# lrjconan/LanczosNetwork

Hardware: AMD Instinct MI355X
Metric: molecules/sec LanczosNet forward, QM8 batch=1024 (higher is better)
Workload: dtype f32; 1 GPU; QM8 LanczosNet batch=1024/GPU, N<=32 dense L (tile N=26), K=20, fp32, 7x128 layers, 1xMI355X per rank; step = [pack L + batch plan + Lanczos + tridiagonal eigensolver (Ritz pairs)] (one launch) + spectral gains + fused forward; global_batch=1024, parallelism=dp1 (batch shards, async score all-gather per step)

## Files before the change

include/lanczosnet_hip.h:

```cpp
#ifndef LANCZOSNET_HIP_H_
#define LANCZOSNET_HIP_H_

#include <stdint.h>

#ifdef __cplusplus
extern "C" {
#endif

#define LNZ_ABI_VERSION 7
#define LNZ_OK 0
#define LNZ_EINVAL (-1)
#define LNZ_ELAUNCH (-2)
#define LNZ_ENOTSUP (-3)

#define LNZ_TILE 32
#define LNZ_MAX_CHANNELS 32
#define LNZ_STRIP_SUB 6
#define LNZ_STRIP_INTS 80
#define LNZ_STRIP_MAX_B 2048

typedef void* lnz_stream_t;

int lnz_abi_version(void);
const char* lnz_last_error(void);
const char* lnz_last_kernel(void);

int lnz_laplacian_l4(const float* adjs, const int32_t* n_nodes, int B, int N, int E,
                     float* L, lnz_stream_t stream);
int lnz_laplacian(const float* adjs, const int32_t* n_nodes, int B, int N, int E, int kind,
                  double alpha, float* L, lnz_stream_t stream);

int lnz_lanczos_ritz(const float* A, int64_t stride_b, int64_t stride_r, int64_t stride_c,
                     const int32_t* n_nodes, int B, int N, int K, float* D, float* V,
                     int32_t* info, lnz_stream_t stream);
// ... 219 lines not shown
  float* dx0;
  int32_t bwd_din0;
  const float* x0;
  float* msg;
  int32_t msg_layer;
  const uint32_t* ident;
  const int64_t* row_off;
  float* dgains;
  float* dy_compact;
  int64_t dy_compact_rows;
  float* dbias_part;
  int32_t dbias_part_cap;
  const int32_t* strips;
  const int32_t* n_strips;
  int strip_cap;
} lnz_forward_args;
int lnz_lanczosnet_forward(const lnz_forward_args* args, lnz_stream_t stream);
int lnz_lanczosnet_input_grad(const lnz_forward_args* args, lnz_stream_t stream);
int lnz_lanczosnet_gain_grad(const lnz_forward_args* args, lnz_stream_t stream);
int lnz_lanczosnet_messages(const lnz_forward_args* args, lnz_stream_t stream);
int lnz_plan_wg_cap(int B, int n_cu);
int lnz_plan_tiles(const uint8_t* mask, int B, int N, int n_cu, int allow_pairs, int32_t* plan,
                   int32_t* n_wg, lnz_stream_t stream);
int lnz_plan_batch(const uint8_t* mask, int B, int N, int n_cu, int allow_pairs, int32_t* plan,
                   int32_t* n_wg, int K, int32_t* gain_rows, int32_t* n_gain_rows,
                   int32_t* strips, int32_t* n_strips, lnz_stream_t stream);
int lnz_strip_cap(int B);
int lnz_plan_strips(const uint8_t* mask, int B, int N, int n_cu, int32_t* strips,
                    int32_t* n_strips, lnz_stream_t stream);
int64_t lnz_head_backward_workspace_floats(int P, int n_wg);
// ... 120 lines not shown
```

lanczosnet_amd/_lib.py:

```python
import ctypes as C
import os

_HERE = os.path.dirname(os.path.abspath(__file__))
LIB_PATH = os.environ.get('LANCZOSNET_HIP_LIB') or os.path.join(_HERE, 'csrc', 'liblanczosnet_hip.so')

LNZ_OK, LNZ_EINVAL, LNZ_ELAUNCH, LNZ_ENOTSUP = 0, -1, -2, -3
ABI_VERSION = 7


class LnzError(RuntimeError):
  def __init__(self, code, msg):
    super().__init__('lanczosnet_hip error %d: %s' % (code, msg))
    self.code = code


class NotSupported(LnzError, NotImplementedError):
  pass


class ForwardArgs(C.Structure):
  _fields_ = [
      ('B', C.c_int32), ('N', C.c_int32), ('K', C.c_int32),
      ('num_layer', C.c_int32),
      ('din0', C.c_int32), ('dhid', C.c_int32), ('dout', C.c_int32),
      ('n_short', C.c_int32), ('n_long', C.c_int32), ('n_edge', C.c_int32),
      ('short_dist', C.c_int32 * 8),
      ('node_feat', C.c_void_p), ('node_feat_f', C.c_void_p), ('embedding', C.c_void_p),
      ('num_atom', C.c_int32), ('filter_kind', C.c_int32),
      ('mask', C.c_void_p), ('Lp', C.c_void_p), ('V', C.c_void_p), ('G', C.c_void_p),
      ('Wp', C.c_void_p), ('bias', C.c_void_p),
      ('w_off', C.c_int64 * 16), ('b_off', C.c_int64 * 16),
      ('Wp_head', C.c_void_p), ('bias_head', C.c_void_p),
      ('score', C.c_void_p), ('state_out', C.c_void_p),
      ('gemm_mode', C.c_int32), ('plan', C.c_void_p), ('n_wg', C.c_void_p), ('plan_wg_cap', C.c_int),
      ('act_out', C.c_void_p), ('act', C.c_void_p), ('dy', C.c_void_p), ('dx0', C.c_void_p),
      ('bwd_din0', C.c_int32), ('x0', C.c_void_p), ('msg', C.c_void_p), ('msg_layer', C.c_int32), ('ident', C.c_void_p), ('row_off', C.c_void_p), ('dgains', C.c_void_p),
      ('dy_compact', C.c_void_p), ('dy_compact_rows', C.c_int64), ('dbias_part', C.c_void_p),
      ('dbias_part_cap', C.c_int32),
      ('strips', C.c_void_p), ('n_strips', C.c_void_p), ('strip_cap', C.c_int),
  ]


_P, _I, _L = C.c_void_p, C.c_int, C.c_int64
SIGNATURES = {
    'lnz_abi_version': (C.c_int, []),
    'lnz_last_error': (C.c_char_p, []),
    'lnz_last_kernel': (C.c_char_p, []),
    'lnz_laplacian_l4': (C.c_int, [_P, _P, _I, _I, _I, _P, _P]),
    'lnz_laplacian': (C.c_int, [_P, _P, _I, _I, _I, _I, C.c_double, _P, _P]),
    'lnz_lanczos_ritz': (C.c_int, [_P, _L, _L, _L, _P, _I, _I, _I, _P, _P, _P, _P]),
    'lnz_lanczos_ritz_workspace_bytes': (C.c_int64, [_I, _I]),
    'lnz_lanczos_ritz_ws': (C.c_int, [_P, _L, _L, _L, _P, _I, _I, _I, _P, _P, _P, _P, _L, _I, _P]),
    'lnz_tridiag_eigh': (C.c_int, [_P, _P, _I, _I, _P, _P, _P]),
    'lnz_lanczos_ritz_large_workspace_bytes': (C.c_int64, [_I, _I]),
# ... 152 lines not shown
```

lanczosnet_amd/csrc/conv_strip.hip:

```cpp
#include "common.hpp"
#include "conv_tiles.hpp"
#include "wave.hpp"
#include <type_traits>

namespace {

constexpr int P = 136;
constexpr int VBP = 20;
constexpr int HP = 33;
constexpr int MAXMOL = 24;
typedef const __attribute__((address_space(3))) float* lds_cptr;
typedef const __attribute__((address_space(3))) f32x4* lds_c4ptr;

__device__ __forceinline__ f32x4 lds4(lds_cptr p) { return *(lds_c4ptr)p; }
__device__ __forceinline__ f32x4 mfma16(float a, float b, f32x4 c) {
  return __builtin_amdgcn_mfma_f32_16x16x4f32(a, b, c, 0, 0, 0);
}
__device__ __forceinline__ f32x4 splat4(float v) { return f32x4{v, v, v, v}; }

typedef _Float16 f16x8 __attribute__((ext_vector_type(8)));
typedef _Float16 f16x4 __attribute__((ext_vector_type(4)));
__device__ __forceinline__ f32x4 mfma32h(f32x4 a, f32x4 b, f32x4 c) {
  return __builtin_amdgcn_mfma_f32_16x16x32_f16(__builtin_bit_cast(f16x8, a), __builtin_bit_cast(f16x8, b),
                                                c, 0, 0, 0);
// ... 53 lines not shown
    const _Float16* g = reinterpret_cast<const _Float16*>(rowp) + half_at(4 * c4);
    const f16x4 h = *reinterpret_cast<const f16x4*>(g), l = *reinterpret_cast<const f16x4*>(g + 32);
    return f32x4{(float)h[0] + (float)l[0], (float)h[1] + (float)l[1], (float)h[2] + (float)l[2],
                 (float)h[3] + (float)l[3]};
  } else {
    return *reinterpret_cast<const f32x4*>(rowp + 4 * c4);
  }
}

constexpr int VH = 512;
constexpr int strip_lds_floats(int S, int nl, bool half = false) {
  return 2 * S * 16 * P + S * 3 * (half ? VH : 16 * VBP) + 2 * nl * S * 16 + 3 * S * 16 + 3 * MAXMOL + 8;
}


template <int S, int MODE, int FK, bool SHORT, bool HALF>
__device__ __forceinline__ void strip_forward(KArgs& a, const int32_t* __restrict__ ent, float* lds,
                                              const int tid, const int wave) {
  constexpr int R = 16 * S;
  constexpr bool FWD = MODE == 0;
  constexpr bool DIAG = FK == 0;
  static_assert(!HALF || (FWD && DIAG && !SHORT), "split precision: inference forward, diagonal gains, no short channels");
#ifdef LNZ_STRIP_PHASES
  long long ph[8] = {0, 0, 0, 0, 0, 0, 0, 0}, t_all = clock64(), _t0 = t_all;
#define LNZ_PH(i) { const long long _t1 = clock64(); ph[i] += _t1 - _t0; _t0 = _t1; }
#else
#define LNZ_PH(i)
#endif
  const int lane = tid & 63;
  const int j = lane & 15, kq = lane >> 4;
  const int N = a.N, K = a.K, B = a.B;
  const int ns = SHORT ? a.n_short : 0, nl = a.n_long, ne = a.n_edge;
  const int C = ns + nl + ne;
  float* Xs = lds;
  float* Vb = Xs + 2 * R * P;
  float* Gs = Vb + S * 3 * (HALF ? VH : 16 * VBP);
  int* rowinfo = reinterpret_cast<int*>(Gs + 2 * nl * R);
// ... 18 lines not shown
      const int n = mext[i];
      const int rows = n <= 4 ? 4 : (n + 3) & ~3;
      if (tid >= mstart[i] && tid < mstart[i] + rows) own = i;
    }
    rowinfo[tid] = own;
    int ok = 0;
    if (own >= 0) {
      const int lrow = tid - mstart[own];
      ok = (lrow < N && a.mask[(int64_t)mid[own] * N + lrow] != 0) ? 1 : 0;
      if (FWD && a.ident) atomicAnd(&idI[tid >> 4], (int)a.ident[mid[own]]);
    }
    rowok[tid] = ok;
  }
  __syncthreads();

  {
    const int d4 = a.din0 >> 2, total = R * d4;
    constexpr int UN = 3;
    for (int base = tid; base < total; base += 512 * UN) {
      int row[UN], c4[UN];
      bool in[UN], valid[UN];
      int64_t at[UN];
#pragma unroll
      for (int u = 0; u < UN; ++u) {
        const int idx = base + 512 * u;
        in[u] = idx < total;
        row[u] = in[u] ? idx / d4 : 0;
        c4[u] = in[u] ? idx - row[u] * d4 : 0;
        const int own = rowinfo[row[u]];
        const int mol = own >= 0 ? mid[own] : 0, lrow = own >= 0 ? row[u] - mstart[own] : 0;
// ... 231 lines not shown
          for (int r = 0; r < 4; ++r)
            xs_put<HALF>(&Xs[nxt * R * P + (16 * I + 4 * kq + r) * P], 16 * wave + j, Y[I][r]);
      }
      __syncthreads();
    }

    LNZ_PH(1)
    f32x4 Z[S], acur[S], alow[HALF ? S : 1];
    auto load_first = [&](lds_cptr x0) {
#pragma unroll
      for (int I = 0; I < S; ++I) {
        acur[I] = lds4(x0 + 16 * I * P);
        if constexpr (HALF) alow[I] = lds4(x0 + 16 * I * P + 16);
      }
    };
    auto steps4 = [&](lds_cptr xb, lds_cptr x0, auto wrap) {
#pragma unroll
      for (int u = 0; u < 4; ++u) {
        ring[(u + 3) & 3] = wp[(u + 3) * 128];
        f32x4 anext[S];
        const lds_cptr xn = (decltype(wrap)::value && u == 3) ? x0 : xb + 16 * (u + 1);
#pragma unroll
        for (int I = 0; I < S; ++I) anext[I] = lds4(xn + 16 * I * P);
        const float4 bv = ring[u];
#pragma unroll
        for (int I = 0; I < S; ++I) Z[I] = mfma16(acur[I][0], bv.x, Z[I]);
#pragma unroll
        for (int I = 0; I < S; ++I) Z[I] = mfma16(acur[I][1], bv.y, Z[I]);
#pragma unroll
        for (int I = 0; I < S; ++I) Z[I] = mfma16(acur[I][2], bv.z, Z[I]);
#pragma unroll
        for (int I = 0; I < S; ++I) Z[I] = mfma16(acur[I][3], bv.w, Z[I]);
#pragma unroll
        for (int I = 0; I < S; ++I) acur[I] = anext[I];
#pragma unroll
        for (int g = 0; g < S; ++g) {
          __builtin_amdgcn_sched_group_barrier(0x008, 3, 0);
          __builtin_amdgcn_sched_group_barrier(0x100, 1, 0);
          if (g == S - 1) __builtin_amdgcn_sched_group_barrier(0x020, 1, 0);
          __builtin_amdgcn_sched_group_barrier(0x008, 1, 0);
        }
      }
      wp += 4 * 128;
    };
    auto gemm1 = [&](lds_cptr x0, auto&& before_last) {
      if (((chan_total ^ (wave >> 2)) & 1) != 0) __builtin_amdgcn_s_setprio(1);
      else __builtin_amdgcn_s_setprio(0);
      ++chan_total;
#pragma unroll
      for (int I = 0; I < S; ++I) Z[I] = splat4(0.f);
      if constexpr (HALF) {
        before_last();
#pragma unroll
        for (int b = 0; b < 4; ++b) {
          f32x4 anext[S], lnext[S];
          const lds_cptr xn = b == 3 ? x0 : x0 + 32 * (b + 1);
#pragma unroll
          for (int I = 0; I < S; ++I) {
            anext[I] = lds4(xn + 16 * I * P);
            lnext[I] = lds4(xn + 16 * I * P + 16);
          }
          const f32x4 bh = __builtin_bit_cast(f32x4, ring[2 * b]);
          const f32x4 bl = __builtin_bit_cast(f32x4, ring[2 * b + 1]);
// ... 10 lines not shown
            acur[I] = anext[I];
            alow[I] = lnext[I];
          }
        }
        wp += 8 * 128;
        return;
      }
      lds_cptr xb = x0;
#pragma unroll 1
      for (int q0 = 4; q0 < Q16; q0 += 4) {
        steps4(xb, x0, std::false_type{});
        xb += 64;
      }
      before_last();
      steps4(xb, x0, std::true_type{});
    };

    f32x4 mop[S][3];
    auto fetch = [&](int e, bool use_ident) {
#pragma unroll
      for (int I = 0; I < S; ++I) {
        const unsigned skip = (use_ident && ((idm[I] >> e) & 1)) ? OOB : 0u;
#pragma unroll
        for (int d = 0; d < 3; ++d) {
          if (I + d - 1 < 0 || I + d - 1 >= S) continue;
          mop[I][d] = __builtin_bit_cast(
              f32x4, __builtin_amdgcn_raw_buffer_load_b128(l_rsrc, loff[I][d] | skip, e * 4096, 0));
        }
      }
    };
// ... 76 lines not shown
#pragma unroll
          for (int I = 0; I < S; ++I) Z[I] = Zn[I];
        }
        apply_all(out, Z);
      }
    }

    if (nl > 0 && active) {
      const lds_cptr y0 = xlane + nxt * R * P;
      load_first(y0);
      f32x4 T[S];
#pragma unroll
      for (int I = 0; I < S; ++I) T[I] = splat4(0.f);
      for (int s = 0; s < nl; ++s) {
        if constexpr (DIAG) {
          gemm1(y0, [] {});
#pragma unroll
          for (int I = 0; I < S; ++I) {
            const f32x4 gv = *reinterpret_cast<const f32x4*>(gsl + s * R + 16 * I + 4 * kq);
            T[I] += gv * Z[I];
          }
        } else {
          gemm1(y0, [&] {
#pragma unroll
            for (int I = 0; I < S; ++I)
#pragma unroll
              for (int d = 0; d < 3; ++d) {
                if (I + d - 1 < 0 || I + d - 1 >= S) continue;
                mop[I][d] = __builtin_bit_cast(
                    f32x4, __builtin_amdgcn_raw_buffer_load_b128(
                               g_rsrc, doff[DIAG ? 0 : I][d], (la * B * nl + s) * K * K * 4, 0));
// ... 19 lines not shown
#pragma unroll
          for (int r = 0; r < 4; ++r)
#pragma unroll
            for (int I = 0; I < S; ++I) {
              const int J = I + d - 1;
              if (J < 0 || J >= S) continue;
              out[I] = mfma16(vl[I][d][r], T[J][r], out[I]);
            }
      }
    }

    LNZ_PH(3)
    if (active) {
      const lds_cptr x0 = xlane + cur * R * P;
      load_first(x0);
      for (int e = 0; e < ne; ++e) {
        gemm1(x0, [&] { fetch(e, true); });
        LNZ_PH(4)
        apply_all(out, Z);
#pragma unroll
        for (int I = 0; I < S; ++I)
          if ((idm[I] >> e) & 1) out[I] += Z[I];
        LNZ_PH(5)
      }
    }

    if (DIAG && nl > 0 && more) store_gains(lg);
    if (nl > 0) __syncthreads();
    if (active) {
      const int col = 16 * wave + j;
#pragma unroll
      for (int I = 0; I < S; ++I) {
        const int row0 = 16 * I + 4 * kq;
        int own = rowinfo[row0];
        asm volatile("" : "+v"(own));
        const int mol = own >= 0 ? mid[own] : 0;
        const int lrow0 = own >= 0 ? row0 - mstart[own] : 0;
        const int64_t rowbase = (int64_t)mol * 32 + lrow0;
// ... 648 lines not shown
  const int tid = threadIdx.x;
  const int wave = __builtin_amdgcn_readfirstlane(tid >> 6);
  const int32_t* ent = a.strips + (int64_t)blockIdx.x * LNZ_STRIP_INTS;
  const int sub = __builtin_amdgcn_readfirstlane(ent[1]);
  switch (sub) {
    case 1: strip_forward<1, MODE, FK, SHORT, HALF>(a, ent, lds_strip, tid, wave); break;
    case 2: strip_forward<2, MODE, FK, SHORT, HALF>(a, ent, lds_strip, tid, wave); break;
    case 3: strip_forward<3, MODE, FK, SHORT, HALF>(a, ent, lds_strip, tid, wave); break;
    case 4: strip_forward<4, MODE, FK, SHORT, HALF>(a, ent, lds_strip, tid, wave); break;
    case 5: strip_forward<5, MODE, FK, SHORT, HALF>(a, ent, lds_strip, tid, wave); break;
    case 6: strip_forward<6, MODE, FK, SHORT, HALF>(a, ent, lds_strip, tid, wave); break;
    default: break;
  }
}

}

namespace lnz {

bool strip_forward_eligible(const lnz_forward_args& a, int mode) {
  if (mode != 0 && mode != 1) return false;
  if (!a.strips || !a.n_strips || a.strip_cap <= 0) return false;
  if (a.filter_kind != 0 && a.filter_kind != 1) return false;
  if (a.gemm_mode == 1 ? (mode != 0 || a.act_out || a.filter_kind != 0 || a.din0 != 128 || a.n_short != 0)
                       : a.gemm_mode != 0)
    return false;
  if (a.dhid != 128 || a.din0 % 64 != 0 || a.din0 > 128) return false;
  if (mode == 1 && (a.din0 != 128 || a.bwd_din0 % 16 != 0)) return false;
  if (mode == 1 && a.dbias_part &&
      a.strip_cap > (a.dbias_part_cap > 0 ? a.dbias_part_cap : (a.plan ? 2 * a.plan_wg_cap : 0)))
    return false;
  if (a.n_short + a.n_long + a.n_edge > 32 || a.n_edge < 1 || a.n_long > 12 || a.dout > 31) return false;
  if (a.filter_kind == 1 && a.K % 4 != 0) return false;
// ... 30 lines not shown
  LNZ_DYNAMIC_LDS(fn, 160 * 1024, "conv_strip.hip");
  lnz_forward_args args = a;
  void* params[] = {&args};
  (void)hipLaunchKernel(fn, dim3(a.strip_cap), dim3(512), params, bytes, s);
  return check_launch("lnz_lanczosnet_messages (strips)");
}

int launch_strip_gain_grad(const lnz_forward_args& a, hipStream_t s) {
  const size_t bytes = (size_t)strip_lds_floats(LNZ_STRIP_SUB, a.n_long) * sizeof(float);
  LNZ_DYNAMIC_LDS(lanczosnet_strip_gain_grad_kernel, 160 * 1024, "conv_strip.hip");
  hipLaunchKernelGGL(lanczosnet_strip_gain_grad_kernel, dim3(a.strip_cap), dim3(512), bytes, s, a);
  return check_launch("lnz_lanczosnet_gain_grad (strips)");
}

int launch_strip_forward(const lnz_forward_args& a, int mode, hipStream_t s) {
  const size_t bytes = (size_t)strip_lds_floats(LNZ_STRIP_SUB, a.n_long, a.gemm_mode == 1) * sizeof(float);
  const void* fns[8] = {
      (const void*)lanczosnet_strip_kernel<0, 0, false>, (const void*)lanczosnet_strip_kernel<1, 0, false>,
      (const void*)lanczosnet_strip_kernel<0, 2, false>, (const void*)lanczosnet_strip_kernel<1, 2, false>,
      (const void*)lanczosnet_strip_kernel<0, 0, true>,  (const void*)lanczosnet_strip_kernel<1, 0, true>,
      (const void*)lanczosnet_strip_kernel<0, 2, true>,  (const void*)lanczosnet_strip_kernel<1, 2, true>};
  const int which = (a.n_short > 0 ? 4 : 0) + (a.filter_kind == 0 ? 0 : 2) + mode;
  const void* fn = fns[which];
  if (a.gemm_mode == 1) fn = (const void*)lanczosnet_strip_kernel<0, 0, false, true>;
  note_kernel("lanczosnet_strip_kernel<%d,%d,%s,%s>", mode, a.filter_kind == 0 ? 0 : 2,
              a.n_short > 0 && a.gemm_mode != 1 ? "true" : "false", a.gemm_mode == 1 ? "true" : "false");
  LNZ_DYNAMIC_LDS(fn, 160 * 1024, "conv_strip.hip");
  lnz_forward_args args = a;
  void* params[] = {&args};
  (void)hipLaunchKernel(fn, dim3(a.strip_cap), dim3(512), params, bytes, s);
  return check_launch(mode == 0 ? "lnz_lanczosnet_forward (strips)" : "lnz_lanczosnet_input_grad (strips)");
// ... 4 lines not shown
```

lanczosnet_amd/csrc/torch_ext.cpp:

```cpp
#include <ATen/ATen.h>
#include <ATen/hip/impl/HIPStreamMasqueradingAsCUDA.h>
#include <c10/core/DeviceGuard.h>
#include <torch/library.h>

#include <tuple>
#include <vector>

#include "../../include/lanczosnet_hip.h"

namespace {

using at::Tensor;

void check(int code, const char* what) {
  TORCH_CHECK(code == LNZ_OK, what, ": lanczosnet_hip error ", code, ": ", lnz_last_error());
}

lnz_stream_t cur_stream() {
  return (lnz_stream_t)c10::hip::getCurrentHIPStreamMasqueradingAsCUDA().stream();
}

void need(const Tensor& t, at::ScalarType dt, const char* name, bool contiguous = true) {
  TORCH_CHECK(t.is_cuda(), "lanczosnet: ", name, " must be a HIP (cuda) tensor; there is no CPU path");
  TORCH_CHECK(t.scalar_type() == dt, "lanczosnet: ", name, " must be ", dt, ", got ", t.scalar_type());
// ... 18 lines not shown
}
void* raw_any(const c10::optional<Tensor>& t, const char* name) {
  if (!t.has_value()) return nullptr;
  TORCH_CHECK(t->is_cuda(), "lanczosnet: ", name, " must be a HIP (cuda) tensor; there is no CPU path");
  return t->data_ptr();
}
const Tensor* first_defined(std::initializer_list<const Tensor*> ts) {
  for (const Tensor* t : ts)
    if (t && t->defined()) return t;
  return nullptr;
}

#include "torch_ext_abi.inc"

enum { kNodeFeat, kNodeFeatF, kEmbedding, kMask, kLp, kV, kG, kWp, kBias, kWpHead, kBiasHead,
       kPlan, kNwg, kAct, kX0, kIdent, kRowOff, kStrips, kNStrips, kNumIn };
enum { dB, dN, dK, dNumLayer, dDin0, dDhid, dDout, dNLong, dNEdge, dNumAtom, dFilterKind, dGemmMode,
       dPlanCap, dBwdDin0, dMsgLayer, dDyCompactRows, dStripCap, kNumDim };
void fused_launch(int64_t which, const c10::List<c10::optional<Tensor>>& in, at::IntArrayRef dims,
                  at::IntArrayRef w_off, at::IntArrayRef b_off,
                  at::IntArrayRef short_dist, const c10::optional<Tensor>& score,
                  const c10::optional<Tensor>& state_out, const c10::optional<Tensor>& act_out,
                  const c10::optional<Tensor>& dy, const c10::optional<Tensor>& dx0,
                  const c10::optional<Tensor>& msg, const c10::optional<Tensor>& dgains,
                  const c10::optional<Tensor>& dy_compact, const c10::optional<Tensor>& dbias_part) {
  TORCH_CHECK((int)in.size() == kNumIn && (int)dims.size() == kNumDim && which >= 0 && which <= 3,
              "lanczosnet::fused_launch: ", (int)kNumIn, " operands and ", (int)kNumDim, " dims expected");
  TORCH_CHECK(w_off.size() <= 16 && b_off.size() <= 16 && short_dist.size() <= 8);
  auto opt = [&](int i) -> c10::optional<Tensor> { return in.get(i); };
  const c10::optional<Tensor> v = opt(kV);
  TORCH_CHECK(v.has_value() && v->dim() == 3, "lanczosnet::fused_launch: V [B,N,K] is required");
  lnz_forward_args a = {};
  a.B = dims[dB], a.N = dims[dN], a.K = dims[dK], a.num_layer = dims[dNumLayer];
// ... 15 lines not shown
  a.V = (const float*)raw_ptr(v, at::kFloat, "V");
  a.G = (const float*)raw_ptr(opt(kG), at::kFloat, "G");
  a.Wp = (const float*)raw_ptr(opt(kWp), at::kFloat, "Wp");
  a.bias = (const float*)raw_ptr(opt(kBias), at::kFloat, "bias");
  a.Wp_head = (const float*)raw_ptr(opt(kWpHead), at::kFloat, "Wp_head");
  a.bias_head = (const float*)raw_ptr(opt(kBiasHead), at::kFloat, "bias_head");
  a.plan = (const int32_t*)raw_ptr(opt(kPlan), at::kInt, "plan");
  a.n_wg = (const int32_t*)raw_ptr(opt(kNwg), at::kInt, "n_wg");
  a.act = (const float*)raw_ptr(opt(kAct), at::kFloat, "act");
  a.x0 = (const float*)raw_ptr(opt(kX0), at::kFloat, "x0");
  a.ident = (const uint32_t*)raw_ptr(opt(kIdent), at::kInt, "ident");
  a.row_off = (const int64_t*)raw_ptr(opt(kRowOff), at::kLong, "row_off");
  a.strips = (const int32_t*)raw_ptr(opt(kStrips), at::kInt, "strips");
  a.n_strips = (const int32_t*)raw_ptr(opt(kNStrips), at::kInt, "n_strips");
  a.strip_cap = dims[dStripCap];
  if (a.strips)
    TORCH_CHECK(a.n_strips && a.strip_cap > 0 &&
                    opt(kStrips)->numel() >= (int64_t)a.strip_cap * LNZ_STRIP_INTS,
                "lanczosnet::fused_launch: strips shorter than strip_cap entries, or n_strips missing");
  if (a.mask) TORCH_CHECK(opt(kMask)->numel() == (int64_t)a.B * a.N, "lanczosnet::fused_launch: mask is not [B,N]");
  if (a.node_feat) TORCH_CHECK(opt(kNodeFeat)->numel() == (int64_t)a.B * a.N, "lanczosnet::fused_launch: node_feat is not [B,N]");
  if (a.node_feat_f)
    TORCH_CHECK(opt(kNodeFeatF)->numel() == (int64_t)a.B * a.N * a.din0, "lanczosnet::fused_launch: node_feat is not [B,N,din0]");
  if (a.G)
    TORCH_CHECK(opt(kG)->numel() == (int64_t)a.num_layer * a.B * a.n_long * a.K * (a.filter_kind == 1 ? a.K : 1) ||
                    opt(kG)->numel() == (int64_t)a.num_layer * a.B * a.n_long * a.K,
                "lanczosnet::fused_launch: G does not match (num_layer, B, n_long, K[, K])");
  if (a.plan) TORCH_CHECK(opt(kPlan)->numel() >= 12 * (int64_t)a.plan_wg_cap, "lanczosnet::fused_launch: plan shorter than 12 * cap");
  a.score = (float*)raw_ptr(score, at::kFloat, "score");
  a.state_out = (float*)raw_ptr(state_out, at::kFloat, "state_out");
// ... 330 lines not shown
```

lanczosnet_amd/ops.py:

```python
import torch

import os
import threading

from . import _lib, _torch_ext



def _map_error(e):
  msg = str(e)
  if 'lanczosnet_hip error ' not in msg:
    return e
  tail = msg.split('lanczosnet_hip error ', 1)[1]
  try:
    code = int(tail.split(':', 1)[0])
  except ValueError:
    return e
  text = tail.split(':', 1)[1].strip() if ':' in tail else tail
  text = text.split('\nException raised from', 1)[0].strip()
  if code == _lib.LNZ_ENOTSUP:
    return _lib.NotSupported(code, text)
  return _lib.LnzError(code, text)


# ... 1386 lines not shown
    strips, scap = _strip_buf(B, mask_u8.device)
    buf.strips = strips
    _abi().plan_batch(mask_u8, B, N, n_cu, 1, buf, buf[12 * cap:], 0, None, None, strips,
                      strips[scap * STRIP_INTS:])
    return buf, cap
  _abi().plan_tiles(mask_u8, B, N, n_cu, int(bool(allow_pairs)), buf,
                                buf[12 * cap:])
  return buf, cap


def pairing_supported(plan):
  return True


def lanczosnet_forward(plan, node_feat, Lp, V, G, mask, return_state=False, tiling='auto',
                       act_out=None, use_ident=True):
  _need_cuda(node_feat, Lp, V, G, mask)
  B, N, K = V.shape
  ready = getattr(Lp, 'ready', None)
  if ready is not None:
    torch.cuda.current_stream(Lp.device).wait_event(ready)
  if plan.get('gemm_mode', 0) == 1:
    Lp = split_laplacian_pack(Lp)
  elif Lp.dtype != torch.float32:
    raise RuntimeError('this Laplacian pack is the float16 form of a split-precision plan (gemm_mode 1): '
                       'the exact kernels read the fp32 pack')
  if act_out is None and not return_state:
    return _forward_ext(plan, node_feat, Lp, V, G, mask, tiling, use_ident)
  ops_, dims = _fused_operands(plan, V)
  emb = None
  if node_feat.dtype in (torch.int64,):
    ops_[_IN['node_feat']] = node_feat.contiguous()
    emb = ops_[_IN['embedding']] = plan['embedding']
    dims[_DIM['num_atom']] = emb.shape[0]
  else:
    nf = node_feat.to(torch.float32)
    if nf.shape[-1] != plan['din0']:
      assert nf.shape[-1] == plan['din0_raw']
      nf = torch.nn.functional.pad(nf, (0, plan['din0'] - nf.shape[-1]))
    ops_[_IN['node_feat_f']] = nf.contiguous()
  mask_u8 = mask.to(torch.uint8).contiguous()
  ops_[_IN['mask']] = mask_u8
  ops_[_IN['Lp']] = Lp
  ident = getattr(Lp, 'ident', None)
  if ident is not None and use_ident:
    ops_[_IN['ident']] = ident
  fk = int(plan.get('filter_kind', 0))
  if G is not None:
    want = (plan['num_layer'], B, plan['n_long'], K) + ((K,) if fk == 1 else ())
    assert tuple(G.shape) == want and G.is_contiguous() and G.dtype == torch.float32, \
        (tuple(G.shape), want)
  ops_[_IN['G']] = G
  ops_[_IN['Wp']], ops_[_IN['bias']] = plan['Wp'], plan['bias']
  ops_[_IN['Wp_head']], ops_[_IN['bias_head']] = plan['Wp_head'], plan['bias_head']
  gemm_mode = int(plan.get('gemm_mode', 0))
  dims[_DIM['gemm_mode']] = gemm_mode
  if isinstance(tiling, tuple):
    tiles, cap = tiling
  elif tiling != 'none':
    assert tiling in ('auto', 'single')
    tiles, cap = plan_tiles(mask_u8, allow_pairs=(tiling == 'auto' and pairing_supported(plan)))
  if tiling != 'none':
    _set_plan(ops_, dims, tiles, cap)
  if gemm_mode == 1 and ops_[_IN['strips']] is None:
    strips = plan_strips(mask_u8)
    scap = (strips.numel() - 1) // STRIP_INTS
    ops_[_IN['strips']], ops_[_IN['n_strips']] = strips, strips[scap * STRIP_INTS:]
    dims[_DIM['strip_cap']] = scap
  score = torch.empty((B, plan['dout']), dtype=torch.float32, device=V.device)
  if act_out is not None:
    assert tuple(act_out.shape) == (plan['num_layer'], B, 32, plan['dhid']) and \
        act_out.is_contiguous() and act_out.dtype == torch.float32
  state = None
  if return_state:
    state = torch.zeros((B, 32, plan['dhid']), dtype=torch.float32, device=V.device)
  nl = plan['num_layer']
  _ext().fused_launch(0, ops_, dims, [int(x) for x in plan['w_off'][:nl]],
                      [int(x) for x in plan['b_off'][:nl]], [int(p) for p in plan['short']],
                      score, state, act_out, None, None, None, None, None, None)
  return (score, state) if return_state else score


_IN = {k: i for i, k in enumerate(
    ['node_feat', 'node_feat_f', 'embedding', 'mask', 'Lp', 'V', 'G', 'Wp', 'bias', 'Wp_head',
     'bias_head', 'plan', 'n_wg', 'act', 'x0', 'ident', 'row_off',
     'strips', 'n_strips'])}
_DIM = {k: i for i, k in enumerate(
    ['B', 'N', 'K', 'num_layer', 'din0', 'dhid', 'dout', 'n_long', 'n_edge', 'num_atom', 'filter_kind',
     'gemm_mode', 'plan_cap', 'bwd_din0', 'msg_layer', 'dy_compact_rows', 'strip_cap'])}


def _fused_operands(plan, V):
  B, N, K = V.shape
  ops_ = [None] * len(_IN)
  ops_[_IN['V']] = _f32c(V)
  dims = [0] * len(_DIM)
  for k, v in (('B', B), ('N', N), ('K', K), ('num_layer', plan['num_layer']), ('din0', plan['din0']),
               ('dhid', plan['dhid']), ('dout', plan['dout']), ('n_long', plan['n_long']),
               ('n_edge', plan['n_edge']), ('filter_kind', int(plan.get('filter_kind', 0)))):
    dims[_DIM[k]] = int(v)
  return ops_, dims


def _set_plan(ops_, dims, tiles, cap):
  ops_[_IN['plan']] = tiles
  ops_[_IN['n_wg']] = tiles[12 * cap:]
  dims[_DIM['plan_cap']] = int(cap)
  strips = getattr(tiles, 'strips', None)
  if strips is not None:
    scap = (strips.numel() - 1) // STRIP_INTS
    ops_[_IN['strips']], ops_[_IN['n_strips']] = strips, strips[scap * STRIP_INTS:]
    dims[_DIM['strip_cap']] = scap


STRIP_INTS = 80


def strip_plan_wanted(B, N):
  return N <= 32


def _strip_buf(B, device):
  scap = _abi().strip_cap(B)
  return torch.empty((scap * STRIP_INTS + 1,), dtype=torch.int32, device=device), scap


def plan_strips(mask_u8, n_cu=None):
  B, N = mask_u8.shape
  n_cu = n_cu or _n_cu(mask_u8.device)
  buf, scap = _strip_buf(B, mask_u8.device)
# ... 477 lines not shown
```

lanczosnet_amd/utils/flop_model.py:

```python
import numpy as np

FLOP_PER_MFMA = 2 * 32 * 32 * 2
FLOP_PER_MFMA16 = 2 * 16 * 16 * 4
FLOP_PER_MOPS_COUNT = 512


def _row_groups(n_a, n_b, split):
  ga = (n_a + 7) >> 3
  gb = ((n_b + 7) >> 3) if n_b > 0 else 0
  return ga + gb if split < 32 else ga


def _subtiles16(n_a, n_b, split):
  mask = (1 << ((n_a + 7) >> 3)) - 1
  if split < 32 and n_b > 0:
    mask |= ((1 << ((n_b + 7) >> 3)) - 1) << (split >> 3)
  return (1 if mask & 3 else 0) + (1 if mask & 12 else 0)


def forward16_selected(cfg):
  hid = cfg['hidden_dim']
  return (len(cfg['short_diffusion_dist']) == 0 and all(h == 128 for h in hid) and
          cfg['input_dim'] % 64 == 0 and cfg['input_dim'] <= 128 and
          len(cfg['long_diffusion_dist']) <= 12)
# ... 148 lines not shown
      useful += (din0 // 16) * 4 * touched
    issued += S * 64
    useful += S * 64
    full = issued
    rows_real += t['rows_real']
    rows_tile += 16 * S
  return dict(tiles=len(strips), mfma_issued=int(issued), mfma_unskipped=int(full),
              flops_issued=int(issued) * FLOP_PER_MFMA16, flops_unskipped=int(full) * FLOP_PER_MFMA16,
              mops_counts=int(issued) * (FLOP_PER_MFMA16 // FLOP_PER_MOPS_COUNT),
              useful_row_frac=rows_real / float(max(1, rows_tile)),
              mfma_in_touched_blocks=int(useful),
              subtiles=int(sum(t['sub'] for t in strips)),
              max_subtiles_per_strip=int(max(t['sub'] for t in strips)))


FLOP_PER_MFMA16X32_F16 = 2 * 16 * 16 * 32


def strip_split_mfma_issued(strips, cfg):
  n_long = len(cfg['long_diffusion_dist'])
  n_edge = cfg['num_bond_type'] + 1
  C = n_long + n_edge
  nl = cfg['num_layer']

  def pairs(S):
    n = 0
    for I in range(S):
      p0 = max(I - 1, 0) >> 1
      n += 1
      if 2 * (p0 + 1) < S and 2 * (p0 + 1) <= I + 1:
# ... 15 lines not shown
```

Measured before the change: 1.342 million molecules/s.

## Fold sparse rare edge channels into one shared GEMM plus low-rank corrections

Adds a strip kernel variant that, per strip, scans the rare edge-type Laplacian channels (channels 2 and up) to find rows that differ from identity. When few rows are touched, it sums the weights of those channels and runs one folded GEMM against X, then adds sparse corrections for the touched rows as 'virtual subtiles' built in LDS. The goal is to skip the full per-channel GEMM and block products for nearly empty bond-type channels. The cost is a per-strip scan of the Laplacian tiles, extra LDS, and a different kernel instantiation; S=6 strips fall back to the old path.

```diff
diff --git a/include/lanczosnet_hip.h b/include/lanczosnet_hip.h
--- a/include/lanczosnet_hip.h
+++ b/include/lanczosnet_hip.h
@@ -18,6 +18,7 @@
 #define LNZ_STRIP_SUB 6
 #define LNZ_STRIP_INTS 80
 #define LNZ_STRIP_MAX_B 2048
+#define LNZ_RARE_DEBUG_INTS 512
 
 typedef void* lnz_stream_t;
 
@@ -267,6 +268,9 @@
   const int32_t* strips;
   const int32_t* n_strips;
   int strip_cap;
+  int32_t* rare_strips;
+  int32_t no_fold;
+  int32_t* rare_debug;
 } lnz_forward_args;
 int lnz_lanczosnet_forward(const lnz_forward_args* args, lnz_stream_t stream);
 int lnz_lanczosnet_input_grad(const lnz_forward_args* args, lnz_stream_t stream);
diff --git a/lanczosnet_amd/_lib.py b/lanczosnet_amd/_lib.py
--- a/lanczosnet_amd/_lib.py
+++ b/lanczosnet_amd/_lib.py
@@ -38,6 +38,7 @@
       ('dy_compact', C.c_void_p), ('dy_compact_rows', C.c_int64), ('dbias_part', C.c_void_p),
       ('dbias_part_cap', C.c_int32),
       ('strips', C.c_void_p), ('n_strips', C.c_void_p), ('strip_cap', C.c_int),
+      ('rare_strips', C.c_void_p), ('no_fold', C.c_int32), ('rare_debug', C.c_void_p),
   ]
 
 
diff --git a/lanczosnet_amd/csrc/conv_strip.hip b/lanczosnet_amd/csrc/conv_strip.hip
--- a/lanczosnet_amd/csrc/conv_strip.hip
+++ b/lanczosnet_amd/csrc/conv_strip.hip
@@ -91,13 +91,19 @@
 }
 
 
-template <int S, int MODE, int FK, bool SHORT, bool HALF>
+constexpr int RARE_MAXV = 8, RARE_MAXF = 5, RARE_MAXS = 5;
+constexpr int rare_lds_floats(int S) {
+  return RARE_MAXV * S * 256 + RARE_MAXV * 16 + 2 * RARE_MAXV + 8 + RARE_MAXF * 16 * S + 8;
+}
+
+template <int S, int MODE, int FK, bool SHORT, bool HALF, bool RARE = false>
 __device__ __forceinline__ void strip_forward(KArgs& a, const int32_t* __restrict__ ent, float* lds,
                                               const int tid, const int wave) {
   constexpr int R = 16 * S;
   constexpr bool FWD = MODE == 0;
   constexpr bool DIAG = FK == 0;
   static_assert(!HALF || (FWD && DIAG && !SHORT), "split precision: inference forward, diagonal gains, no short channels");
+  static_assert(!RARE || (FWD && DIAG && !SHORT && !HALF && S <= RARE_MAXS), "rare form: exact inference forward, S <= 5");
 #ifdef LNZ_STRIP_PHASES
   long long ph[8] = {0, 0, 0, 0, 0, 0, 0, 0}, t_all = clock64(), _t0 = t_all;
 #define LNZ_PH(i) { const long long _t1 = clock64(); ph[i] += _t1 - _t0; _t0 = _t1; }
@@ -146,6 +152,143 @@
   }
   __syncthreads();
 
+  float* rx = lds + strip_lds_floats(S, nl);
+  f32x4* Af = reinterpret_cast<f32x4*>(rx);
+  int* vsrc = reinterpret_cast<int*>(rx + RARE_MAXV * S * 256);
+  int* vchan = vsrc + RARE_MAXV * 16;
+  int* tcnt = vchan + 2 * RARE_MAXV;
+  int* tlist = tcnt + 8;
+  int* rflag = tlist + RARE_MAXF * R;
+  bool rare = false;
+  int nvs = 0;
+  if constexpr (RARE) {
+    const int NF = ne - 2;
+    constexpr int TCAP = RARE_MAXF * MAXMOL;
+    unsigned* tmask = reinterpret_cast<unsigned*>(rx);
+    int* tiles = reinterpret_cast<int*>(tmask + TCAP);
+    int* ntile = tiles + TCAP;
+    if (tid < TCAP) tmask[tid] = 0u;
+    if (tid < 2) ntile[tid] = 0;
+    __syncthreads();
+    if (tid < nm * NF) {
+      const int own = tid / NF, f = tid - own * NF;
+      if (a.ident && ((a.ident[mid[own]] >> (2 + f)) & 1u)) tiles[TCAP - 1 - atomicAdd(ntile + 1, 1)] = own * 8 + f;
+      else tiles[atomicAdd(ntile, 1)] = own * 8 + f;
+    }
+    __syncthreads();
+    {
+      const int whole = ntile[0] * 256, total = whole + ntile[1] * 32;
+      constexpr int UN = 4;
+      for (int base = tid; base < total; base += 512 * UN) {
+        float4 v[UN];
+        int tl[UN], o[UN];
+#pragma unroll
+        for (int u = 0; u < UN; ++u) {
+          const int idx = base + 512 * u;
+          tl[u] = -1, o[u] = 0;
+          if (idx < whole) {
+            tl[u] = tiles[idx >> 8], o[u] = idx & 255;
+          } else if (idx < total) {
+            const int jd = idx - whole, r = jd & 31;
+            tl[u] = tiles[TCAP - 1 - (jd >> 5)], o[u] = (r >> 3) * 64 + ((r >> 2) & 1) * 32 + r;
+          }
+          const int64_t at = tl[u] >= 0 ? ((int64_t)mid[tl[u] >> 3] * ne + 2 + (tl[u] & 7)) * 256 + o[u] : 0;
+          v[u] = reinterpret_cast<const float4*>(a.Lp)[at];
+        }
+#pragma unroll
+        for (int u = 0; u < UN; ++u) {
+          if (tl[u] < 0) continue;
+          const int own = tl[u] >> 3;
+          const int row = o[u] & 31, col0 = 8 * (o[u] >> 6) + 4 * ((o[u] >> 5) & 1);
+          const float x[4] = {v[u].x, v[u].y, v[u].z, v[u].w};
+          const int n = mext[own], rows_own = n <= 4 ? 4 : (n + 3) & ~3;
+          unsigned bits = 0u;
+#pragma unroll
+          for (int c = 0; c < 4; ++c) {
+            if (col0 + c != row) bits |= x[c] != 0.0f ? (1u << row) | (1u << (col0 + c)) : 0u;
+            else if (row < rows_own && x[c] != (rowok[mstart[own] + row] != 0 ? 1.0f : 0.0f)) bits |= 1u << row;
+          }
+          if (bits) atomicOr(&tmask[(tl[u] & 7) * MAXMOL + own], bits);
+        }
+      }
+    }
+    __syncthreads();
+    if (wave < NF) {
+      int base = 0;
+      for (int h = 0; h < 2; ++h) {
+        const int row = lane + 64 * h;
+        bool t = false;
+        if (row < R) {
+          const int own = rowinfo[row];
+          if (own >= 0) t = (tmask[wave * MAXMOL + own] >> (row - mstart[own])) & 1;
+        }
+        const unsigned long long m = __ballot(t);
+        if (t) tlist[wave * R + base + __popcll(m & ((1ull << lane) - 1ull))] = row;
+        base += __popcll(m);
+      }
+      if (lane == 0) tcnt[wave] = base;
+    }
+    __syncthreads();
+    if (tid == 0) {
+      int nv = 0;
+      for (int f = 0; f < NF; ++f)
+        for (int s0 = 0; s0 < tcnt[f]; s0 += 16) {
+          if (nv < RARE_MAXV) vchan[nv] = 2 + f, vchan[RARE_MAXV + nv] = s0;
+          ++nv;
+        }
+      const int folded = 32 * S + nv * (32 + 4 * S), plain = (32 * S + 4 * (3 * S - 2)) * NF;
+      rflag[0] = (nv <= RARE_MAXV && folded < plain) ? 1 : 0;
+      rflag[1] = nv;
+    }
+    __syncthreads();
+    rare = __builtin_amdgcn_readfirstlane(rflag[0]) != 0;
+    nvs = rare ? __builtin_amdgcn_readfirstlane(rflag[1]) : 0;
+    if (a.rare_debug) {
+      int32_t* dbg = a.rare_debug + (int64_t)blockIdx.x * LNZ_RARE_DEBUG_INTS;
+      if (tid == 0) dbg[0] = rflag[0], dbg[1] = rflag[1];
+      if (tid < NF) dbg[2 + tid] = tcnt[tid];
+      if (tid < RARE_MAXV && tid < rflag[1]) dbg[8 + tid] = vchan[tid];
+      for (int idx = tid; idx < NF * R; idx += 512) {
+        const int f = idx / R, i = idx - f * R;
+        if (i < tcnt[f]) dbg[16 + 96 * f + i] = tlist[idx];
+      }
+    }
+    if (rare) {
+      if (tid == 0 && a.rare_strips) atomicAdd(a.rare_strips, 1);
+      if (tid < nvs * 16) {
+        const int v = tid >> 4, f = vchan[v] - 2, s0 = vchan[RARE_MAXV + v], slot = s0 + (tid & 15);
+        vsrc[tid] = tlist[f * R + (slot < tcnt[f] ? slot : s0)];
+      }
+      __syncthreads();
+      for (int idx = tid; idx < nvs * S * 64; idx += 512) {
+        const int v = idx / (S * 64), rem = idx - v * (S * 64);
+        const int I = rem >> 6, jj = rem & 15, kk = (rem >> 4) & 3;
+        const int e = vchan[v], f = e - 2, s0 = vchan[RARE_MAXV + v];
+        const int p = 16 * I + jj, own = rowinfo[p];
+        float val[4];
+        bool ok[4];
+        int q[4];
+#pragma unroll
+        for (int r = 0; r < 4; ++r) {
+          const int slot = 4 * kk + r;
+          q[r] = vsrc[v * 16 + slot];
+          ok[r] = s0 + slot < tcnt[f] && own >= 0 && rowinfo[q[r]] == own;
+          int64_t at = 0;
+          if (ok[r]) {
+            const int st = mstart[own], lp = p - st, lq = q[r] - st;
+            at = ((((int64_t)mid[own] * ne + e) * 256 + (lq >> 3) * 64 + ((lq >> 2) & 1) * 32 + lp) << 2) + (lq & 3);
+          }
+          val[r] = a.Lp[at];
+        }
+        f32x4 d;
+#pragma unroll
+        for (int r = 0; r < 4; ++r)
+          d[r] = ok[r] ? val[r] - ((q[r] == p && rowok[p] != 0) ? 1.0f : 0.0f) : 0.0f;
+        Af[idx] = d;
+      }
+    }
+  }
+
   {
     const int d4 = a.din0 >> 2, total = R * d4;
     constexpr int UN = 3;
@@ -407,10 +550,32 @@
         if constexpr (HALF) alow[I] = lds4(x0 + 16 * I * P + 16);
       }
     };
+    const float4* __restrict__ wnext = wp;
+    const float4* __restrict__ wjump = nullptr;
+    f32x4 wf[8];
+    float4 wft[RARE_MAXF];
+    int gi = 0;
+    auto fold_load = [&](int q) {
+#pragma unroll
+      for (int f = 0; f < RARE_MAXF; ++f) {
+        const int e = 2 + f < ne ? 2 + f : ne - 1;
+        wft[f] = Wl[((int64_t)rt * Gtot + (int64_t)(ns + nl + e) * Q) * 64 + wlane + q * 128];
+      }
+    };
+    auto fold_add = [&](int q) {
+      f32x4 sum = splat4(0.f);
+#pragma unroll
+      for (int f = 0; f < RARE_MAXF; ++f)
+        if (2 + f < ne) sum += f32x4{wft[f].x, wft[f].y, wft[f].z, wft[f].w};
+#pragma unroll
+      for (int qq = 0; qq < 8; ++qq)
+        if (qq == q) wf[qq] = sum;
+    };
     auto steps4 = [&](lds_cptr xb, lds_cptr x0, auto wrap) {
 #pragma unroll
       for (int u = 0; u < 4; ++u) {
-        ring[(u + 3) & 3] = wp[(u + 3) * 128];
+        if (RARE && decltype(wrap)::value && u >= 1) ring[(u + 3) & 3] = wnext[(u - 1) * 128];
+        else ring[(u + 3) & 3] = wp[(u + 3) * 128];
         f32x4 anext[S];
         const lds_cptr xn = (decltype(wrap)::value && u == 3) ? x0 : xb + 16 * (u + 1);
 #pragma unroll
@@ -440,6 +605,10 @@
       if (((chan_total ^ (wave >> 2)) & 1) != 0) __builtin_amdgcn_s_setprio(1);
       else __builtin_amdgcn_s_setprio(0);
       ++chan_total;
+      if constexpr (RARE) {
+        wnext = wjump ? wjump : wp + Q16 * 128;
+        wjump = nullptr;
+      }
 #pragma unroll
       for (int I = 0; I < S; ++I) Z[I] = splat4(0.f);
       if constexpr (HALF) {
@@ -480,6 +649,14 @@
       }
       before_last();
       steps4(xb, x0, std::true_type{});
+      if constexpr (RARE) wp = wnext;
+    };
+    auto gemm1_carry = [&](lds_cptr x0, auto&& before_last) {
+      const bool carry = RARE && rare && gi < Q16;
+      if (carry) fold_load(gi);
+      gemm1(x0, before_last);
+      if (carry) fold_add(gi);
+      ++gi;
     };
 
     f32x4 mop[S][3];
@@ -586,7 +763,8 @@
       for (int I = 0; I < S; ++I) T[I] = splat4(0.f);
       for (int s = 0; s < nl; ++s) {
         if constexpr (DIAG) {
-          gemm1(y0, [] {});
+          if constexpr (RARE) gemm1_carry(y0, [] {});
+          else gemm1(y0, [] {});
 #pragma unroll
           for (int I = 0; I < S; ++I) {
             const f32x4 gv = *reinterpret_cast<const f32x4*>(gsl + s * R + 16 * I + 4 * kq);
@@ -636,14 +814,94 @@
     if (active) {
       const lds_cptr x0 = xlane + cur * R * P;
       load_first(x0);
-      for (int e = 0; e < ne; ++e) {
-        gemm1(x0, [&] { fetch(e, true); });
+      const int ne_plain = (RARE && rare) ? 2 : ne;
+      auto wchan = [&](int v) {
+        const int e = __builtin_amdgcn_readfirstlane(vchan[v]);
+        return Wl + ((int64_t)rt * Gtot + (int64_t)(ns + nl + e) * Q) * 64 + wlane;
+      };
+      for (int e = 0; e < ne_plain; ++e) {
+        if constexpr (RARE) {
+          if (rare && e == 1 && nvs > 0) wjump = wchan(0);
+          gemm1_carry(x0, [&] { fetch(e, true); });
+        } else {
+          gemm1(x0, [&] { fetch(e, true); });
+        }
         LNZ_PH(4)
         apply_all(out, Z);
 #pragma unroll
         for (int I = 0; I < S; ++I)
           if ((idm[I] >> e) & 1) out[I] += Z[I];
         LNZ_PH(5)
+      }
+      if constexpr (RARE) {
+        if (rare) {
+          for (int q = gi; q < Q16; ++q) {
+            fold_load(q);
+            fold_add(q);
+          }
+          if (((chan_total ^ (wave >> 2)) & 1) != 0) __builtin_amdgcn_s_setprio(1);
+          else __builtin_amdgcn_s_setprio(0);
+          ++chan_total;
+#pragma unroll
+          for (int I = 0; I < S; ++I) Z[I] = splat4(0.f);
+#pragma unroll
+          for (int q = 0; q < 8; ++q) {
+            if (q < Q16) {
+              f32x4 av[S];
+#pragma unroll
+              for (int I = 0; I < S; ++I) av[I] = lds4(x0 + 16 * q + 16 * I * P);
+#pragma unroll
+              for (int c = 0; c < 4; ++c)
+#pragma unroll
+                for (int I = 0; I < S; ++I) Z[I] = mfma16(av[I][c], wf[q][c], Z[I]);
+            }
+          }
+#pragma unroll
+          for (int I = 0; I < S; ++I) {
+            const int4 okv = *reinterpret_cast<const int4*>(rowok + 16 * I + 4 * kq);
+            out[I][0] += okv.x ? Z[I][0] : 0.0f;
+            out[I][1] += okv.y ? Z[I][1] : 0.0f;
+            out[I][2] += okv.z ? Z[I][2] : 0.0f;
+            out[I][3] += okv.w ? Z[I][3] : 0.0f;
+          }
+          LNZ_PH(4)
+          for (int v = 0; v < nvs; ++v) {
+            if (((chan_total ^ (wave >> 2)) & 1) != 0) __builtin_amdgcn_s_setprio(1);
+            else __builtin_amdgcn_s_setprio(0);
+            ++chan_total;
+            const float4* __restrict__ wn = v + 1 < nvs ? wchan(v + 1) : wp;
+            const lds_cptr xa = (lds_cptr)(Xs + cur * R * P + vsrc[v * 16 + j] * P + 4 * kq);
+            f32x4 zg[4] = {splat4(0.f), splat4(0.f), splat4(0.f), splat4(0.f)};
+            f32x4 ac = lds4(xa);
+#pragma unroll 1
+            for (int q0 = 0; q0 < Q16; q0 += 4) {
+              const bool last = q0 + 4 >= Q16;
+#pragma unroll
+              for (int u = 0; u < 4; ++u) {
+                const float4* pf = (last && u >= 1) ? wn + (u - 1) * 128 : wp + (u + 3) * 128;
+                ring[(u + 3) & 3] = *pf;
+                const f32x4 an = lds4(xa + 16 * ((q0 + u + 1) & (Q16 - 1)));
+                const float4 bv = ring[u];
+                zg[0] = mfma16(ac[0], bv.x, zg[0]);
+                zg[1] = mfma16(ac[1], bv.y, zg[1]);
+                zg[2] = mfma16(ac[2], bv.z, zg[2]);
+                zg[3] = mfma16(ac[3], bv.w, zg[3]);
+                ac = an;
+              }
+              wp += 4 * 128;
+            }
+            wp = wn;
+            const f32x4 zs = (zg[0] + zg[1]) + (zg[2] + zg[3]);
+            f32x4 fr[S];
+#pragma unroll
+            for (int I = 0; I < S; ++I) fr[I] = Af[(v * S + I) * 64 + lane];
+#pragma unroll
+            for (int r = 0; r < 4; ++r)
+#pragma unroll
+              for (int I = 0; I < S; ++I) out[I] = mfma16(fr[I][r], zs[r], out[I]);
+          }
+          LNZ_PH(5)
+        }
       }
     }
 
@@ -1322,9 +1580,37 @@
   }
 }
 
+template <int MODE, int FK, int RARE, bool SHORT, bool HALF>
+__global__ __launch_bounds__(512) void lanczosnet_strip_kernel(const lnz_forward_args) {
+  static_assert(MODE == 0 && FK == 0 && RARE == 1 && !SHORT && !HALF, "one instantiation");
+  KArgs& a = *(KArgs*)__builtin_amdgcn_kernarg_segment_ptr();
+  extern __shared__ __attribute__((aligned(16))) float lds_strip[];
+  if ((int)blockIdx.x >= *a.n_strips) return;
+  const int tid = threadIdx.x;
+  const int wave = __builtin_amdgcn_readfirstlane(tid >> 6);
+  const int32_t* ent = a.strips + (int64_t)blockIdx.x * LNZ_STRIP_INTS;
+  const int sub = __builtin_amdgcn_readfirstlane(ent[1]);
+  switch (sub) {
+    case 1: strip_forward<1, 0, 0, false, false, true>(a, ent, lds_strip, tid, wave); break;
+    case 2: strip_forward<2, 0, 0, false, false, true>(a, ent, lds_strip, tid, wave); break;
+    case 3: strip_forward<3, 0, 0, false, false, true>(a, ent, lds_strip, tid, wave); break;
+    case 4: strip_forward<4, 0, 0, false, false, true>(a, ent, lds_strip, tid, wave); break;
+    case 5: strip_forward<5, 0, 0, false, false, true>(a, ent, lds_strip, tid, wave); break;
+    case 6: strip_forward<6, 0, 0, false, false>(a, ent, lds_strip, tid, wave); break;
+    default: break;
+  }
+}
+
 }
 
 namespace lnz {
+
+static bool strip_rare_eligible(const lnz_forward_args& a, int mode) {
+  if (mode != 0 || a.act_out || a.no_fold) return false;
+  if (a.gemm_mode != 0 || a.filter_kind != 0 || a.n_short != 0) return false;
+  if (a.n_edge < 3 || a.n_edge - 2 > RARE_MAXF) return false;
+  return (size_t)(strip_lds_floats(RARE_MAXS, a.n_long) + rare_lds_floats(RARE_MAXS)) * sizeof(float) <= 160 * 1024;
+}
 
 bool strip_forward_eligible(const lnz_forward_args& a, int mode) {
   if (mode != 0 && mode != 1) return false;
@@ -1385,7 +1671,19 @@
 }
 
 int launch_strip_forward(const lnz_forward_args& a, int mode, hipStream_t s) {
-  const size_t bytes = (size_t)strip_lds_floats(LNZ_STRIP_SUB, a.n_long, a.gemm_mode == 1) * sizeof(float);
+  size_t bytes = (size_t)strip_lds_floats(LNZ_STRIP_SUB, a.n_long, a.gemm_mode == 1) * sizeof(float);
+  if (strip_rare_eligible(a, mode)) {
+    const size_t rb = (size_t)(strip_lds_floats(RARE_MAXS, a.n_long) + rare_lds_floats(RARE_MAXS)) * sizeof(float);
+    bytes = rb > bytes ? rb : bytes;
+    void (*kfn)(const lnz_forward_args) = lanczosnet_strip_kernel<0, 0, 1, false, false>;
+    const void* fn = (const void*)kfn;
+    note_kernel("lanczosnet_strip_kernel<0,0,1,false,false>");
+    LNZ_DYNAMIC_LDS(fn, 160 * 1024, "conv_strip.hip");
+    lnz_forward_args args = a;
+    void* params[] = {&args};
+    (void)hipLaunchKernel(fn, dim3(a.strip_cap), dim3(512), params, bytes, s);
+    return check_launch("lnz_lanczosnet_forward (strips, folded rare channels)");
+  }
   const void* fns[8] = {
       (const void*)lanczosnet_strip_kernel<0, 0, false>, (const void*)lanczosnet_strip_kernel<1, 0, false>,
       (const void*)lanczosnet_strip_kernel<0, 2, false>, (const void*)lanczosnet_strip_kernel<1, 2, false>,
diff --git a/lanczosnet_amd/csrc/torch_ext.cpp b/lanczosnet_amd/csrc/torch_ext.cpp
--- a/lanczosnet_amd/csrc/torch_ext.cpp
+++ b/lanczosnet_amd/csrc/torch_ext.cpp
@@ -56,9 +56,9 @@
 #include "torch_ext_abi.inc"
 
 enum { kNodeFeat, kNodeFeatF, kEmbedding, kMask, kLp, kV, kG, kWp, kBias, kWpHead, kBiasHead,
-       kPlan, kNwg, kAct, kX0, kIdent, kRowOff, kStrips, kNStrips, kNumIn };
+       kPlan, kNwg, kAct, kX0, kIdent, kRowOff, kStrips, kNStrips, kRareStrips, kRareDebug, kNumIn };
 enum { dB, dN, dK, dNumLayer, dDin0, dDhid, dDout, dNLong, dNEdge, dNumAtom, dFilterKind, dGemmMode,
-       dPlanCap, dBwdDin0, dMsgLayer, dDyCompactRows, dStripCap, kNumDim };
+       dPlanCap, dBwdDin0, dMsgLayer, dDyCompactRows, dStripCap, dNoFold, kNumDim };
 void fused_launch(int64_t which, const c10::List<c10::optional<Tensor>>& in, at::IntArrayRef dims,
                   at::IntArrayRef w_off, at::IntArrayRef b_off,
                   at::IntArrayRef short_dist, const c10::optional<Tensor>& score,
@@ -104,6 +104,12 @@
   a.strips = (const int32_t*)raw_ptr(opt(kStrips), at::kInt, "strips");
   a.n_strips = (const int32_t*)raw_ptr(opt(kNStrips), at::kInt, "n_strips");
   a.strip_cap = dims[dStripCap];
+  a.rare_strips = (int32_t*)raw_ptr(opt(kRareStrips), at::kInt, "rare_strips");
+  a.no_fold = (int32_t)dims[dNoFold];
+  a.rare_debug = (int32_t*)raw_ptr(opt(kRareDebug), at::kInt, "rare_debug");
+  if (a.rare_debug)
+    TORCH_CHECK(opt(kRareDebug)->numel() >= (int64_t)dims[dStripCap] * LNZ_RARE_DEBUG_INTS,
+                "lanczosnet::fused_launch: rare_debug shorter than strip_cap * LNZ_RARE_DEBUG_INTS");
   if (a.strips)
     TORCH_CHECK(a.n_strips && a.strip_cap > 0 &&
                     opt(kStrips)->numel() >= (int64_t)a.strip_cap * LNZ_STRIP_INTS,
diff --git a/lanczosnet_amd/ops.py b/lanczosnet_amd/ops.py
--- a/lanczosnet_amd/ops.py
+++ b/lanczosnet_amd/ops.py
@@ -1424,7 +1424,8 @@
 
 
 def lanczosnet_forward(plan, node_feat, Lp, V, G, mask, return_state=False, tiling='auto',
-                       act_out=None, use_ident=True):
+                       act_out=None, use_ident=True, rare_strips=None, fold=True,
+                       rare_debug=None):
   _need_cuda(node_feat, Lp, V, G, mask)
   B, N, K = V.shape
   ready = getattr(Lp, 'ready', None)
@@ -1435,7 +1436,7 @@
   elif Lp.dtype != torch.float32:
     raise RuntimeError('this Laplacian pack is the float16 form of a split-precision plan (gemm_mode 1): '
                        'the exact kernels read the fp32 pack')
-  if act_out is None and not return_state:
+  if act_out is None and not return_state and rare_strips is None and rare_debug is None and fold:
     return _forward_ext(plan, node_feat, Lp, V, G, mask, tiling, use_ident)
   ops_, dims = _fused_operands(plan, V)
   emb = None
@@ -1455,6 +1456,12 @@
   ident = getattr(Lp, 'ident', None)
   if ident is not None and use_ident:
     ops_[_IN['ident']] = ident
+  if rare_strips is not None:
+    assert rare_strips.dtype == torch.int32 and rare_strips.numel() >= 1
+    ops_[_IN['rare_strips']] = rare_strips
+  if rare_debug is not None:
+    assert rare_debug.dtype == torch.int32 and rare_debug.is_contiguous()
+    ops_[_IN['rare_debug']] = rare_debug
   fk = int(plan.get('filter_kind', 0))
   if G is not None:
     want = (plan['num_layer'], B, plan['n_long'], K) + ((K,) if fk == 1 else ())
@@ -1465,6 +1472,7 @@
   ops_[_IN['Wp_head']], ops_[_IN['bias_head']] = plan['Wp_head'], plan['bias_head']
   gemm_mode = int(plan.get('gemm_mode', 0))
   dims[_DIM['gemm_mode']] = gemm_mode
+  dims[_DIM['no_fold']] = 0 if fold else 1
   if isinstance(tiling, tuple):
     tiles, cap = tiling
   elif tiling != 'none':
@@ -1494,10 +1502,10 @@
 _IN = {k: i for i, k in enumerate(
     ['node_feat', 'node_feat_f', 'embedding', 'mask', 'Lp', 'V', 'G', 'Wp', 'bias', 'Wp_head',
      'bias_head', 'plan', 'n_wg', 'act', 'x0', 'ident', 'row_off',
-     'strips', 'n_strips'])}
+     'strips', 'n_strips', 'rare_strips', 'rare_debug'])}
 _DIM = {k: i for i, k in enumerate(
     ['B', 'N', 'K', 'num_layer', 'din0', 'dhid', 'dout', 'n_long', 'n_edge', 'num_atom', 'filter_kind',
-     'gemm_mode', 'plan_cap', 'bwd_din0', 'msg_layer', 'dy_compact_rows', 'strip_cap'])}
+     'gemm_mode', 'plan_cap', 'bwd_din0', 'msg_layer', 'dy_compact_rows', 'strip_cap', 'no_fold'])}
 
 
 def _fused_operands(plan, V):
@@ -1524,6 +1532,7 @@
 
 
 STRIP_INTS = 80
+RARE_DEBUG_INTS = 512
 
 
 def strip_plan_wanted(B, N):
diff --git a/lanczosnet_amd/utils/flop_model.py b/lanczosnet_amd/utils/flop_model.py
--- a/lanczosnet_amd/utils/flop_model.py
+++ b/lanczosnet_amd/utils/flop_model.py
@@ -186,6 +186,91 @@
               max_subtiles_per_strip=int(max(t['sub'] for t in strips)))
 
 
+RARE_MAXV, RARE_MAXF, RARE_MAXS = 8, 5, 5
+
+
+def touch_masks(L, mask):
+  L = np.asarray(L, np.float32)
+  B, N = L.shape[:2]
+  off = L != 0.0
+  eye = np.eye(N, dtype=bool)[None, :, :, None]
+  off = off & ~eye
+  t = off.any(axis=2) | off.any(axis=1)
+  diag = np.einsum('biic->bic', L)
+  t |= diag != (np.asarray(mask) != 0).astype(np.float32)[:, :, None]
+  bits = (np.uint64(1) << np.arange(N, dtype=np.uint64))[None, :, None]
+  return (t * bits).sum(axis=1).astype(np.uint32)
+
+
+def strip_touch_counts(strips, touch, n_edge):
+  p = np.asarray(strips)
+  cap = (p.size - 1) // STRIP_INTS
+  out = []
+  for s in range(int(p[cap * STRIP_INTS])):
+    e = p[s * STRIP_INTS:(s + 1) * STRIP_INTS]
+    cnt = [0] * max(0, n_edge - 2)
+    for i in range(int(e[0])):
+      b, _, n = (int(x) for x in e[2 + 3 * i:5 + 3 * i])
+      rows = 4 if n <= 4 else (n + 3) // 4 * 4
+      for f in range(len(cnt)):
+        cnt[f] += bin(int(touch[b][2 + f]) & ((1 << rows) - 1)).count('1')
+    out.append(cnt)
+  return out
+
+
+def rare_cost(S, touch_count, n_fold):
+  nv = sum((c + 15) // 16 for c in touch_count)
+  return 32 * S + nv * (32 + 4 * S), (32 * S + 4 * (3 * S - 2)) * n_fold, nv
+
+
+def strip_takes_rare(S, touch_count, n_fold):
+  if S > RARE_MAXS or n_fold < 1 or n_fold > RARE_MAXF:
+    return False
+  folded, plain, nv = rare_cost(S, touch_count, n_fold)
+  return nv <= RARE_MAXV and folded < plain
+
+
+def strip_rare_mfma_issued(strips, touch_counts, cfg):
+  n_long = len(cfg['long_diffusion_dist'])
+  n_edge = cfg['num_bond_type'] + 1
+  C = n_long + n_edge
+  n_fold = n_edge - 2
+  din0, dhid, nl = cfg['input_dim'], cfg['hidden_dim'][0], cfg['num_layer']
+  din0 = (din0 + 63) // 64 * 64
+  issued = plain = 0
+  rare_strips = nvt = 0
+  per_layer = []
+  for i, t in enumerate(strips):
+    S = t['sub']
+    blocks = 3 * S - 2
+    tc = touch_counts[i] if touch_counts is not None else None
+    rare = tc is not None and strip_takes_rare(S, tc, n_fold)
+    nv = rare_cost(S, tc, n_fold)[2] if rare else 0
+    rare_strips += int(rare)
+    nvt += nv
+    for l in range(nl):
+      d_in = din0 if l == 0 else dhid
+      proj = 1 if (n_long and l + 1 < nl) else 0
+      blk = 4 * blocks * ((1 if n_long else 0) + proj)
+      old = C * (d_in // 16) * 4 * S + blk + 4 * n_edge * blocks
+      new = old if not rare else ((n_long + 3) * (d_in // 16) * 4 * S + nv * ((d_in // 16) * 4 + 4 * S) +
+                                  blk + 4 * 2 * blocks)
+      issued += 8 * new
+      plain += 8 * old
+      if l == 1:
+        per_layer.append((S, new))
+    extra = ((din0 // 16) * 4 * blocks if n_long else 0) + S * 64
+    issued += extra
+    plain += extra
+  smax = max(t['sub'] for t in strips)
+  top = [c for s, c in per_layer if s == smax]
+  return dict(tiles=len(strips), mfma_issued=int(issued), mfma_channel_loop=int(plain),
+              flops_issued=int(issued) * FLOP_PER_MFMA16,
+              mops_counts=int(issued) * (FLOP_PER_MFMA16 // FLOP_PER_MOPS_COUNT),
+              rare_strips=rare_strips, virtual_subtiles=nvt,
+              per_wave_layer_worst=int(max(top)), per_wave_layer_mean=float(np.mean(top)))
+
+
 FLOP_PER_MFMA16X32_F16 = 2 * 16 * 16 * 32
 
 
```

After: 1.450 million molecules/s, median of 6. +8.1%, better.
